# skipperro/selkies-gstreamer

Hardware: AMD Instinct MI355X
Metric: encoded fps + glass-to-glass p50 ms at 1920x1080; concurrent 60fps sessions/node (higher is better)
Workload: dtype uint8 pixels / int32 integer transforms (bit-exact vs CPU reference); 1 GPU; model=H.264 Constrained Baseline CAVLC, striped stripes 64px, CRF 25, global_batch=8, seq_len=1, parallelism=session-parallel dp1 x 8 sessions/GPU, resolution=1920x1080, backend=hip, deblock=auto, me_full=True, upload_overlap=False, frames_in_flight=1, num_refs=1, numa_node_rank0=0

## Files before the change

### csrc/kernels/h264_gpu.h

```cpp
#pragma once
#include <hip/hip_runtime.h>
#include "../codec/overlay.h"
#include "../codec/h264_encoder.h"
#include "../codec/h264_frame.h"
#include "../codec/h264_deblock.h"

namespace sk {
namespace h264 {
namespace gpu {

constexpr int kMbSlotBytes = 1024;
constexpr int kSliceHdrMax = 64;

struct Planes {
    uint8_t* y;
    uint8_t* u;
    uint8_t* v;
};

struct FrameArgs {
    int W, H, mb_w, mb_h, stride_y, stride_c, num_slices, rows_per_slice, fullframe;
    int full_range, me_range, me_iters;
    const uint8_t* bgrx;
    int bgrx_stride;
// ... 7 lines not shown
    int* plan_ctl;
    const int* key_seq_host;
    int* key_dev;
    PlanConfig plan_cfg;
    SliceTask* tasks;
    MeResult* me;
    int16_t* mvfield;
    MbInfo* mbs;
    int16_t* coefs;
    uint32_t* mb_bits;
    int* mb_nbits;
    uint32_t* rbsp;
    int rbsp_slot_words;
    int* mb_off;
    int* slice_info;
    int* tile_nz;
    int* tile_ins;
    int max_tiles;
    int out_slot_bytes;
    const uint8_t* param_sets;
    const int* param_set_len;
    int param_set_stride;
    uint8_t* host_out;
    int* host_size;
    int* frame_params_dev;
    const int* frame_params_host;
    SliceTask* tasks_host;
    unsigned long long* dbg;
    const CavlcTables* cavlc_tabs;
    int num_refs;
    int deblock;
// ... 32 lines not shown
```

### csrc/kernels/h264_kernels.hip

```cpp
#include "h264_gpu.h"
#include "../codec/color.h"
#include "../codec/h264_mb.h"

namespace sk {
namespace h264 {
namespace gpu {

__device__ __forceinline__ int lane_id() { return threadIdx.x & 63; }

__device__ __forceinline__ void wave_sync() {
    __builtin_amdgcn_fence(__ATOMIC_RELEASE, "wavefront");
    __builtin_amdgcn_wave_barrier();
    __builtin_amdgcn_fence(__ATOMIC_ACQUIRE, "wavefront");
}

__device__ __forceinline__ int wave_sum(int v) {
    v += __builtin_amdgcn_mov_dpp(v, 0xB1, 0xF, 0xF, false);
    v += __builtin_amdgcn_mov_dpp(v, 0x4E, 0xF, 0xF, false);
    v += __builtin_amdgcn_mov_dpp(v, 0x124, 0xF, 0xF, false);
    v += __builtin_amdgcn_mov_dpp(v, 0x128, 0xF, 0xF, false);
    return __builtin_amdgcn_readlane(v, 0) + __builtin_amdgcn_readlane(v, 16) +
           __builtin_amdgcn_readlane(v, 32) + __builtin_amdgcn_readlane(v, 48);
}

// ... 313 lines not shown

__device__ __forceinline__ uint32_t load_ref4(const uint8_t* row, int x, int stride) {
    if (x >= 0 && x + 3 <= stride - 1) {
        int xa = x & ~3, sh = x & 3;
        uint32_t w0 = *reinterpret_cast<const uint32_t*>(row + xa);
        if (sh == 0) return w0;
        uint32_t w1 = *reinterpret_cast<const uint32_t*>(row + xa + 4);
        return __builtin_amdgcn_alignbyte(w1, w0, sh);
    }
    uint32_t v = 0;
#pragma unroll
    for (int i = 0; i < 4; i++) v |= (uint32_t)row[sk_clip(x + i, 0, stride - 1)] << (8 * i);
    return v;
}

__device__ __forceinline__ int me_sad(const FrameArgs& a, const uint8_t* refy, uint32_t sw, int mbx,
                                      int mby, int dx, int dy, int ylo, int yhi) {
    int l = lane_id();
    int row = l >> 2, col4 = (l & 3) * 4;
    int sy = sk_clip(mby * 16 + row + dy, ylo, yhi);
    uint32_t rw = load_ref4(refy + (size_t)sy * a.stride_y, mbx * 16 + col4 + dx, a.stride_y);
    return wave_sum((int)__builtin_amdgcn_sad_u8(sw, rw, 0u));
}

constexpr int kWin = 8;
constexpr int kWinWords = 10;

__device__ __forceinline__ uint32_t win_sad_lane(const uint32_t* win, uint32_t sw, int ox, int oy) {
    const int l = lane_id();
    const int row = l >> 2, col4 = (l & 3) * 4;
    const int bc = col4 + ox + kWin;
    const uint32_t* w = win + (row + oy + kWin) * kWinWords + (bc >> 2);
    const int sh = bc & 3;
    const uint32_t rw = sh ? __builtin_amdgcn_alignbyte(w[1], w[0], sh) : w[0];
    return __builtin_amdgcn_sad_u8(sw, rw, 0u);
}

__device__ __forceinline__ int win_sad(const uint32_t* win, uint32_t sw, int ox, int oy) {
    const int l = lane_id();
    const int row = l >> 2, col4 = (l & 3) * 4;
    const int bc = col4 + ox + kWin;
    const uint32_t* w = win + (row + oy + kWin) * kWinWords + (bc >> 2);
    const int sh = bc & 3;
    const uint32_t rw = sh ? __builtin_amdgcn_alignbyte(w[1], w[0], sh) : w[0];
    return wave_sum((int)__builtin_amdgcn_sad_u8(sw, rw, 0u));
}

__device__ __forceinline__ int mb_activity(uint32_t sw) {
    const int psum = (int)(sw & 255) + (int)((sw >> 8) & 255) + (int)((sw >> 16) & 255) + (int)(sw >> 24);
    const int mean = (wave_sum(psum) + 128) >> 8;
    int dev = 0;
#pragma unroll
    for (int i = 0; i < 4; i++) dev += sk_abs((int)((sw >> (8 * i)) & 255) - mean);
    return wave_sum(dev);
}

__global__ __launch_bounds__(64) void k_motion_search(FrameArgs a) {
    __shared__ uint32_t win[32 * kWinWords];
    int nmb = a.mb_w * a.mb_h;
    int idx = xcd_remap(blockIdx.x, gridDim.x);
    if (idx >= nmb) return;
    int mbx = idx % a.mb_w, mby = idx / a.mb_w;
    int s = mby / a.rows_per_slice;
    const SliceTask t = a.tasks[s];
    if (t.action != ACT_P && t.action != ACT_I) return;
    int l = lane_id();
    int row = l >> 2, col4 = (l & 3) * 4;
    uint32_t sw = *reinterpret_cast<const uint32_t*>(a.src.y + (size_t)(mby * 16 + row) * a.stride_y +
                                                     mbx * 16 + col4);
    if (t.action == ACT_I) {
        const int dev = mb_activity(sw);
        if (l == 0) a.me[idx] = MeResult{0, 0, 0, dev, 0, 0, 0};
        return;
    }
    int ylo = t.pic_row0 * 16, yhi = (t.pic_row0 + t.pic_rows) * 16 - 1;
    const int lam = lambda_for_qp(rc_me_qp(*a.rc, t.qp));
    const int R = a.me_range;
    int cx[7], cy[7], n = 0;
    cx[0] = 0; cy[0] = 0; n = 1;
    auto add = [&](int ox, int oy) {
        int j = oy * a.mb_w + ox;
        cx[n] = sk_clip(a.mvfield[2 * j], -R, R);
        cy[n] = sk_clip(a.mvfield[2 * j + 1], -R, R);
        n++;
    };
    add(mbx, mby);
    if (mbx > 0) add(mbx - 1, mby);
    if (mbx + 1 < a.mb_w) add(mbx + 1, mby);
    if (mby - 1 >= t.pic_row0) add(mbx, mby - 1);
    if (mby + 1 < t.pic_row0 + t.pic_rows) add(mbx, mby + 1);
    if (a.me_full && a.mb_dirty[idx]) {
        cx[n] = sk_clip(a.fs_mv[2 * idx], -R, R);
        cy[n] = sk_clip(a.fs_mv[2 * idx + 1], -R, R);
        n++;
    }
    int bx = 0, by = 0;
    int bsad = me_sad(a, a.ref.y, sw, mbx, mby, 0, 0, ylo, yhi);
    int bcost = bsad + lam * (sk_se_bits(0) + sk_se_bits(0));
    for (int i = 1; i < n; i++) {
        int sd = me_sad(a, a.ref.y, sw, mbx, mby, cx[i], cy[i], ylo, yhi);
        int c = sd + lam * (sk_se_bits(4 * cx[i]) + sk_se_bits(4 * cy[i]));
        if (c < bcost) { bcost = c; bx = cx[i]; by = cy[i]; bsad = sd; }
    }
    const int cx0 = bx, cy0 = by;
    {
        const int r = l >> 1, h = l & 1;
        const int y = sk_clip(mby * 16 + cy0 - kWin + r, ylo, yhi);
        const uint8_t* rowp = a.ref.y + (size_t)y * a.stride_y;
        const int x0 = mbx * 16 + cx0 - kWin + 16 * h;
#pragma unroll
        for (int k = 0; k < 5; k++) win[r * kWinWords + 4 * h + k] = load_ref4(rowp, x0 + 4 * k, a.stride_y);
    }
    wave_sync();
    const int ddx[4] = {0, -1, 1, 0}, ddy[4] = {-1, 0, 0, 1};
    for (int it = 0; it < a.me_iters; it++) {
        int nb = -1, ncost = bcost, nsad = 0;
        bool all_in = true;
#pragma unroll
        for (int k = 0; k < 4; k++) {
            const int ox = bx + ddx[k] - cx0, oy = by + ddy[k] - cy0;
            all_in = all_in && ox >= -kWin && ox <= kWin && oy >= -kWin && oy <= kWin;
        }
        if (all_in) {
            uint32_t p[4];
#pragma unroll
            for (int k = 0; k < 4; k++) p[k] = win_sad_lane(win, sw, bx + ddx[k] - cx0, by + ddy[k] - cy0);
            const uint32_t s01 = (uint32_t)wave_sum((int)(p[0] | (p[1] << 16)));
            const uint32_t s23 = (uint32_t)wave_sum((int)(p[2] | (p[3] << 16)));
            const int sds[4] = {(int)(s01 & 0xffff), (int)(s01 >> 16), (int)(s23 & 0xffff), (int)(s23 >> 16)};
#pragma unroll
            for (int k = 0; k < 4; k++) {
                int x = bx + ddx[k], y = by + ddy[k];
                if (x < -R || x > R || y < -R || y > R) continue;
                int c = sds[k] + lam * (sk_se_bits(4 * x) + sk_se_bits(4 * y));
                if (c < ncost) { ncost = c; nb = k; nsad = sds[k]; }
            }
            if (nb < 0) break;
            bx += ddx[nb]; by += ddy[nb]; bcost = ncost; bsad = nsad;
            continue;
        }
#pragma unroll
        for (int k = 0; k < 4; k++) {
            int x = bx + ddx[k], y = by + ddy[k];
            if (x < -R || x > R || y < -R || y > R) continue;
            const int ox = x - cx0, oy = y - cy0;
            int sd = (ox >= -kWin && ox <= kWin && oy >= -kWin && oy <= kWin)
                         ? win_sad(win, sw, ox, oy)
                         : me_sad(a, a.ref.y, sw, mbx, mby, x, y, ylo, yhi);
            int c = sd + lam * (sk_se_bits(4 * x) + sk_se_bits(4 * y));
            if (c < ncost) { ncost = c; nb = k; nsad = sd; }
        }
        if (nb < 0) break;
        bx += ddx[nb]; by += ddy[nb]; bcost = ncost; bsad = nsad;
    }
    const int dev = mb_activity(sw);
    int refi = 0;
    if (t.num_refs > 1 && a.mb_dirty[idx]) {
        const int s1 = me_sad(a, a.ref1.y, sw, mbx, mby, 0, 0, ylo, yhi);
        if (s1 + 3 * lam < bcost) {
            bx = by = 0;
            bsad = s1;
            refi = 1;
        }
    }
    if (l == 0) {
        MeResult r;
        r.mvx = (int16_t)bx;
        r.mvy = (int16_t)by;
        r.sad = bsad;
        r.intra_est = dev;
        r.ref = (int16_t)refi;
        r.fx = r.fy = 0;
        a.me[idx] = r;
    }
}

typedef int v4i __attribute__((ext_vector_type(4)));

__global__ __launch_bounds__(256) void k_me_mfma(FrameArgs a) {
    constexpr int WW = kFsWin / 4;
    constexpr int WP = WW + 1;
    constexpr int BP = 5;
    constexpr int SP = 2 * kFsR + 4;
    __shared__ uint32_t win_s[4][kFsWin * WP];
    __shared__ uint32_t blk_s[4][16 * BP];
    __shared__ __align__(16) int sq_s[4][kFsWin * SP];
    const int w = threadIdx.x >> 6, l = lane_id();
    const int nmb = a.mb_w * a.mb_h;
    const int idx = xcd_remap(blockIdx.x, gridDim.x) * 4 + w;
    if (idx >= nmb) return;
    const int mbx = idx % a.mb_w, mby = idx / a.mb_w;
    const SliceTask t = a.tasks[mby / a.rows_per_slice];
    if (t.action != ACT_P || !a.mb_dirty[idx]) return;
    const int ylo = t.pic_row0 * 16, yhi = (t.pic_row0 + t.pic_rows) * 16 - 1;
    {
        const int R = a.me_range;
        const int px = sk_clip(a.mvfield[2 * idx], -R, R), py = sk_clip(a.mvfield[2 * idx + 1], -R, R);
        const uint32_t sw = *reinterpret_cast<const uint32_t*>(a.src.y + (size_t)(mby * 16 + (l >> 2)) * a.stride_y +
                                                               mbx * 16 + (l & 3) * 4);
        if (me_sad(a, a.ref.y, sw, mbx, mby, px, py, ylo, yhi) == 0) {
            if (l == 0) {
                a.fs_mv[2 * idx] = (int16_t)px;
                a.fs_mv[2 * idx + 1] = (int16_t)py;
            }
            return;
        }
    }
    uint32_t* win = win_s[w];
    uint32_t* blk = blk_s[w];
    int* sq = sq_s[w];
    for (int i = l; i < kFsWin * WW; i += 64) {
        const int wy = i / WW, q = i - wy * WW;
        const int y = sk_clip(mby * 16 - kFsR + wy, ylo, yhi);
        win[wy * WP + q] = load_ref4(a.ref.y + (size_t)y * a.stride_y, mbx * 16 - kFsR + 4 * q, a.stride_y);
    }
    blk[(l >> 2) * BP + (l & 3)] = *reinterpret_cast<const uint32_t*>(a.src.y + (size_t)(mby * 16 + (l >> 2)) * a.stride_y +
                                                                     mbx * 16 + (l & 3) * 4);
    wave_sync();
    if (l < kFsWin) {
        uint32_t rw[WW];
#pragma unroll
        for (int q = 0; q < WW; q++) rw[q] = win[l * WP + q];
        int sqv[kFsWin];
#pragma unroll
        for (int c = 0; c < kFsWin; c++) {
            const int v = (int)((rw[c >> 2] >> (8 * (c & 3))) & 255) - 128;
            sqv[c] = v * v;
        }
        int acc = 0;
#pragma unroll
        for (int c = 0; c < 16; c++) acc += sqv[c];
        int out[2 * kFsR];
        out[0] = acc;
#pragma unroll
        for (int x = 1; x < 2 * kFsR; x++) {
            acc += sqv[x + 15] - sqv[x - 1];
            out[x] = acc;
        }
#pragma unroll
        for (int x = 0; x < 2 * kFsR; x += 4)
            *reinterpret_cast<int4*>(&sq[l * SP + x]) = make_int4(out[x], out[x + 1], out[x + 2], out[x + 3]);
    }
    wave_sync();
    if (l < 2 * kFsR) {
        int col[kFsWin];
#pragma unroll
        for (int r = 0; r < kFsWin; r++) col[r] = sq[r * SP + l];
        int acc = 0;
#pragma unroll
        for (int r = 0; r < 16; r++) acc += col[r];
#pragma unroll
        for (int dy = 0; dy < 2 * kFsR; dy++) {
            sq[dy * SP + l] = acc;
            acc += col[dy + 16] - col[dy];
        }
    }
    const int i16 = l & 15, g = l >> 4;
    v4i acc[2][2];
#pragma unroll
    for (int mt = 0; mt < 2; mt++)
#pragma unroll
        for (int nt = 0; nt < 2; nt++) acc[mt][nt] = v4i{0, 0, 0, 0};
#pragma unroll
    for (int ks = 0; ks < kFsWin / 4; ks++) {
        const int rr = 4 * ks + g;
        v4i bf[2];
#pragma unroll
        for (int nt = 0; nt < 2; nt++) {
            const int src = rr - (16 * nt + i16);
            const bool in = src >= 0 && src < 16;
#pragma unroll
            for (int q = 0; q < 4; q++) bf[nt][q] = in ? (int)(blk[(in ? src : 0) * BP + q] ^ 0x80808080u) : 0;
        }
#pragma unroll
        for (int mt = 0; mt < 2; mt++) {
            const int b0 = 16 * mt + i16;
            const uint32_t* wr = win + rr * WP + (b0 >> 2);
            const int sh = b0 & 3;
            uint32_t w5[5];
#pragma unroll
            for (int q = 0; q < 5; q++) w5[q] = wr[q];
            v4i af;
#pragma unroll
            for (int q = 0; q < 4; q++) af[q] = (int)(__builtin_amdgcn_alignbyte(w5[q + 1], w5[q], sh) ^ 0x80808080u);
#pragma unroll
            for (int nt = 0; nt < 2; nt++)
                if (ks >= 4 * nt && ks <= 4 * nt + 7)
                    acc[mt][nt] = __builtin_amdgcn_mfma_i32_16x16x64_i8(af, bf[nt], acc[mt][nt], 0, 0, 0);
        }
    }
    wave_sync();
    uint64_t best = ~0ull;
#pragma unroll
    for (int mt = 0; mt < 2; mt++)
#pragma unroll
        for (int nt = 0; nt < 2; nt++) {
            const int dyw = 16 * nt + i16;
            const int4 sv = *reinterpret_cast<const int4*>(&sq[dyw * SP + 16 * mt + 4 * g]);
            const int svr[4] = {sv.x, sv.y, sv.z, sv.w};
#pragma unroll
            for (int reg = 0; reg < 4; reg++) {
                const int dxw = 16 * mt + 4 * g + reg;
                const uint64_t k = fs_key(svr[reg] - 2 * acc[mt][nt][reg], dyw, dxw);
                best = k < best ? k : best;
            }
        }
#pragma unroll
    for (int o = 1; o < 64; o <<= 1) {
        const uint64_t other = __shfl_xor(best, o);
        best = other < best ? other : best;
    }
    if (l == 0) {
        a.fs_mv[2 * idx] = (int16_t)fs_key_dx(best);
        a.fs_mv[2 * idx + 1] = (int16_t)fs_key_dy(best);
    }
}

__global__ __launch_bounds__(256) void k_plan(FrameArgs a) {
    const int ns = a.num_slices, tid = threadIdx.x;
    StripeState* st = a.plan_state;
    StripeState& pic = st[ns];
    if (a.plan_ctl[1] == 1) {
        if (a.fullframe) {
            bool idr = true;
            for (int s = tid; s < ns; s += 256) idr &= a.tasks[s].final_action == ACT_I && a.tasks[s].idr_on_intra;
            idr = __syncthreads_and(idr);
            if (tid == 0) commit_picture(pic, idr, a.plan_cfg.num_refs);
        } else {
            for (int s = tid; s < ns; s += 256) commit_stripe(st[s], a.tasks[s].final_action, a.plan_cfg.num_refs);
        }
// ... 88 lines not shown
                rc.last_bits[k] = old.last_bits[k];
                rc.last_cplx[k] = old.last_cplx[k];
            }
        if (old.mode == mode) rc.cplx_ema = old.cplx_ema;
        rc.seq = seq;
    }
    rc.base_qp = plan_qp;
    rc_apply(rc, a.tasks, a.rc_slice, a.rc_slice + 1, a.num_slices, a.mb_w, plan_qp, 2);
}
__global__ __launch_bounds__(64) void k_rc_qp(FrameArgs a) {
    if (threadIdx.x == 0) rc_qp_serial(a);
    __syncthreads();
    for (int s = threadIdx.x; s < a.num_slices; s += 64) a.tasks_host[s].qp = a.tasks[s].qp;
}

__global__ __launch_bounds__(64) void k_rc_account(FrameArgs a, const int* sizes, int n, int stride, int per_slice) {
    long long b = 0;
    for (int i = threadIdx.x; i < n; i += 64)
        if (!per_slice || i % per_slice < slice_nals(a, a.tasks[i / per_slice])) b += sizes[(size_t)i * stride];
    for (int o = 32; o > 0; o >>= 1) b += __shfl_down(b, o);
    if (threadIdx.x == 0) rc_account(*a.rc, 8 * b);
}

__global__ __launch_bounds__(256) void k_rc_guard(FrameArgs a) {
    __shared__ long long part[4];
    const int s = blockIdx.x, tid = threadIdx.x;
    long long b = 0;
    for (int i = tid; i < a.num_slices; i += 256) {
        const int nn = slice_nals(a, a.tasks[i]);
        for (int j = 0; j < nn; j++) b += a.slice_info[4 * (i * a.nal_per_slice + j)];
    }
    for (int o = 32; o > 0; o >>= 1) b += __shfl_down(b, o);
    if ((tid & 63) == 0) part[tid >> 6] = b;
    __syncthreads();
    const long long bits = 8 * (part[0] + part[1] + part[2] + part[3]);
    const int step = rc_redo_step(*a.rc, bits);
// ... 1654 lines not shown
            uint32_t hi = 0u;
            if (k >= 1) {
                hi = src[k - 1];
                if (k - 1 == nw - 1) hi &= lastmask;
            }
            v = (lo >> sh) | (k >= 1 ? hi << (32 - sh) : 0u);
        }
        if (j == w0 || j == w1) {
            if (v) atomicOr(&dst[j], v);
        } else {
            dst[j] = v;
        }
    }
}

__device__ __forceinline__ uint8_t rbsp_byte(uint32_t word, int q) { return (uint8_t)(word >> (24 - 8 * q)); }

__global__ __launch_bounds__(256) void k_ep_nz(FrameArgs a) {
    __shared__ int red[4];
    const int s = blockIdx.y, t = blockIdx.x, tid = threadIdx.x;
    const int nn = slice_nals(a, a.tasks[s]);
    for (int j = 0; j < nn; j++) {
    const int nal = s * a.nal_per_slice + j;
    const int n = a.slice_info[4 * nal];
    const int t0 = t * kTile;
    if (t0 >= n) continue;
    const uint32_t* rbsp = nal_rbsp(a, s, j);
    const int i0 = t0 + tid * 16;
    int lastnz = -1;
#pragma unroll
    for (int q = 0; q < 4; q++) {
        const int iq = i0 + 4 * q;
        const uint32_t wd = iq < n ? rbsp[iq >> 2] : 0u;
#pragma unroll
        for (int b = 0; b < 4; b++)
            if (iq + b < n && rbsp_byte(wd, b)) lastnz = iq + b;
    }
    for (int o = 32; o > 0; o >>= 1) lastnz = max(lastnz, __shfl_down(lastnz, o));
    if (lane_id() == 0) red[tid >> 6] = lastnz;
    __syncthreads();
    if (tid == 0) a.tile_nz[nal * a.max_tiles + t] = max(max(red[0], red[1]), max(red[2], red[3]));
    __syncthreads();
    }
}

__device__ __forceinline__ int ep_thread(const uint32_t* rbsp, int n, int t0, int carry, int* scan_lds,
                                         uint8_t* by, uint32_t* insmask) {
    const int tid = threadIdx.x, wv = tid >> 6, ln = tid & 63;
    const int i0 = t0 + tid * 16;
    int lastnz = -1;
#pragma unroll
    for (int q = 0; q < 4; q++) {
        const int iq = i0 + 4 * q;
        const uint32_t wd = iq < n ? rbsp[iq >> 2] : 0u;
#pragma unroll
        for (int j = 0; j < 4; j++) {
            by[4 * q + j] = rbsp_byte(wd, j);
            if (iq + j < n && by[4 * q + j]) lastnz = iq + j;
        }
    }
    const int incl = wave_incl_scan_max(lastnz);
    int ex = __shfl_up(incl, 1);
    if (ln == 0) ex = -1;
    if (ln == 63) scan_lds[wv] = incl;
    __syncthreads();
    int prev = carry;
    for (int k = 0; k < wv; k++) prev = max(prev, scan_lds[k]);
    prev = max(prev, ex);
    int ins = 0;
    uint32_t mask = 0;
#pragma unroll
    for (int q = 0; q < 16; q++) {
        const int i = i0 + q;
        if (i < n) {
            const int z = i - 1 - prev;
            if (by[q] <= 3 && z >= 2 && !(z & 1)) {
                ins++;
                mask |= 1u << q;
            }
            if (by[q]) prev = i;
        }
    }
    *insmask = mask;
    return ins;
}

__device__ __forceinline__ int tile_carry(const FrameArgs& a, int nal, int t) {
    int c = -1;
    for (int k = 0; k < t; k++) c = max(c, a.tile_nz[nal * a.max_tiles + k]);
    return c;
}

__global__ __launch_bounds__(256) void k_ep_count(FrameArgs a) {
    __shared__ int scan_lds[4];
    __shared__ int red[4];
    const int s = blockIdx.y, t = blockIdx.x;
    const int nn = slice_nals(a, a.tasks[s]);
    for (int j = 0; j < nn; j++) {
        const int nal = s * a.nal_per_slice + j;
        const int n = a.slice_info[4 * nal];
        const int t0 = t * kTile;
        if (t0 >= n) continue;
        const uint32_t* rbsp = nal_rbsp(a, s, j);
        uint8_t by[16];
        uint32_t mask;
        int ins = ep_thread(rbsp, n, t0, tile_carry(a, nal, t), scan_lds, by, &mask);
        for (int o = 32; o > 0; o >>= 1) ins += __shfl_down(ins, o);
        if (lane_id() == 0) red[threadIdx.x >> 6] = ins;
        __syncthreads();
        if (threadIdx.x == 0) a.tile_ins[nal * a.max_tiles + t] = red[0] + red[1] + red[2] + red[3];
        __syncthreads();
    }
}

__global__ __launch_bounds__(256) void k_ep_write(FrameArgs a) {
    __shared__ int scan_lds[4];
    __shared__ int wave_tot[5];
    __shared__ int sh_before, sh_base;
    __shared__ uint8_t sOut[kTile + kTile / 2 + 16];
    const int s = blockIdx.y, t = blockIdx.x, tid = threadIdx.x;
    const SliceTask& task = a.tasks[s];
// ... 10 lines not shown
        int base = 0;
        for (int jj = 0; jj < j; jj++) {
            const int q = s * a.nal_per_slice + jj, nq = a.slice_info[4 * q];
            int ins_q = 0;
            for (int k = tid; k * kTile < nq; k += 64) ins_q += a.tile_ins[q * a.max_tiles + k];
            base += a.slice_info[4 * q + 1] + nq + wave_sum(ins_q);
        }
        if (tid == 0) {
            sh_before = b;
            sh_base = base;
        }
    }
    uint32_t* rbsp = nal_rbsp(a, s, j);
    uint8_t by[16];
    uint32_t mask;
    const int ins = ep_thread(rbsp, n, t0, tile_carry(a, nal, t), scan_lds, by, &mask);
    int tile_ins;
    const int ex = block_excl_scan<4>(ins, wave_tot, &tile_ins);
    const int i0 = t0 + tid * 16;
    int o = tid * 16 + ex;
#pragma unroll
    for (int q = 0; q < 16; q++) {
        if (i0 + q < n) {
            if (mask & (1u << q)) sOut[o++] = 3;
            sOut[o++] = by[q];
        }
    }
#pragma unroll
    for (int q = 0; q < 4; q++)
        if (i0 + 4 * q < n) rbsp[(i0 >> 2) + q] = 0u;
    __syncthreads();
// ... 319 lines not shown
            }
        }
        lds_barrier();
    }
}

void launch_convert_damage(const FrameArgs& a, hipStream_t s) {
    dim3 grid((a.mb_w + 15) / 16, a.mb_h);
    if (a.yuv_fmt) hipLaunchKernelGGL(k_yuv_damage, grid, dim3(256), 0, s, a);
    else hipLaunchKernelGGL(k_convert_damage, grid, dim3(256), 0, s, a);
}

void launch_frontend(const FrameArgs& a, hipStream_t s) {
    int nmb = a.mb_w * a.mb_h;
    hipLaunchKernelGGL(k_plan, dim3(1), dim3(256), 0, s, a);
    if (a.me_full) hipLaunchKernelGGL(k_me_mfma, dim3((nmb + 3) / 4), dim3(256), 0, s, a);
    hipLaunchKernelGGL(k_motion_search, dim3(nmb), dim3(64), 0, s, a);
    hipLaunchKernelGGL(k_decide, dim3(a.num_slices), dim3(256), 0, s, a);
    hipLaunchKernelGGL(k_rc_qp, dim3(1), dim3(64), 0, s, a);
    if (a.subpel) hipLaunchKernelGGL(k_subpel, dim3((nmb + 3) / 4), dim3(256), 0, s, a);
}

void launch_rc_guard_sizes(const FrameArgs& a, const int* sizes, int n, int* redo, bool chained, hipStream_t s) {
    hipLaunchKernelGGL(k_rc_guard_sizes, dim3(1), dim3(256), 0, s, a, sizes, n, redo, chained ? 1 : 0);
}

void launch_rc_account(const FrameArgs& a, const int* sizes, int n, int stride, int per_slice, hipStream_t s) {
    hipLaunchKernelGGL(k_rc_account, dim3(1), dim3(64), 0, s, a, sizes, n, stride, per_slice);
}

static void launch_code(const FrameArgs& a, hipStream_t s) {
    int nmb = a.mb_w * a.mb_h;
// ... 10 lines not shown
}

void launch_encode(const FrameArgs& a, hipStream_t s, bool guard) {
    int nmb = a.mb_w * a.mb_h;
    launch_frontend(a, s);
    if (a.aq_strength > 0) hipLaunchKernelGGL(k_aq, dim3((nmb + 3) / 4), dim3(256), 0, s, a);
    launch_code(a, s);
    if (guard && a.rc_redo) {
        hipLaunchKernelGGL(k_rc_guard, dim3(a.num_slices), dim3(256), 0, s, a);
        FrameArgs b = a;
        b.gate = a.rc_redo;
        launch_code(b, s);
    }
    hipLaunchKernelGGL(k_mb_concat, dim3((nmb + 3) / 4), dim3(256), 0, s, a);
    const dim3 tiles(a.max_tiles, a.num_slices);
    hipLaunchKernelGGL(k_ep_nz, tiles, dim3(256), 0, s, a);
    hipLaunchKernelGGL(k_ep_count, tiles, dim3(256), 0, s, a);
    hipLaunchKernelGGL(k_ep_write, tiles, dim3(256), 0, s, a);
    launch_rc_account(a, a.slice_info, a.num_slices * a.nal_per_slice, 4, a.nal_per_slice, s);
}

void launch_commit(const FrameArgs& a, hipStream_t s) {
    hipLaunchKernelGGL(k_commit, dim3((a.mb_w + 15) / 16, a.mb_h), dim3(256), 0, s, a);
    if (a.deblock) {
        const int nmb = a.mb_w * a.mb_h;
        hipLaunchKernelGGL(k_deblock_prep, dim3((nmb + 3) / 4), dim3(256), 0, s, a);
        hipLaunchKernelGGL(k_deblock_edges, dim3((nmb + 255) / 256), dim3(256), 0, s, a);
        if (a.rows_per_slice <= 4)
            hipLaunchKernelGGL(k_deblock<4>, dim3(a.num_slices), dim3(64 * a.rows_per_slice), 0, s, a);
        else
            hipLaunchKernelGGL(k_deblock<kMaxRows>, dim3(a.num_slices), dim3(64 * a.rows_per_slice), 0, s, a);
    }
}

// ... 4 lines not shown
```

### csrc/runtime/h264_hip.cpp

```cpp
#include "encoder_iface.h"
#include "trace.h"
#include "../kernels/h264_gpu.h"
#include "../kernels/hevc_gpu.h"
#include "../kernels/av1_gpu.h"
#include "../codec/av1_encoder.h"
#include "../kernels/runtime_kernels.h"
#include "../codec/hevc_encoder.h"
#include <hip/hip_runtime.h>
#include <atomic>
#include <chrono>
#include <map>
#include <mutex>
#include <stdexcept>
#include <string.h>
#include <string>
#include <thread>
#include <vector>
#include <atomic>

namespace sk {
namespace {

#define HIPCHECK(x)                                                                     \
    do {                                                                                \
// ... 530 lines not shown
        a.dbe = dmalloc<uint4>((size_t)3 * nmb);
        a.mbs = dmalloc<MbInfo>(nmb);
        a.coefs = dmalloc<int16_t>((size_t)nmb * kCoefPerMb);
        a.mb_bits = dmalloc<uint32_t>((size_t)nmb * (gpu::kMbSlotBytes / 4));
        a.mb_nbits = dmalloc<int>(nmb);
        int max_slice_mbs = g_.rows_per_slice * g_.mb_w;
        const bool can_split = cfg_.codec == 0 && g_.mb_w > kIntraSubMbs;
        a.nal_per_slice = can_split ? max_nals_per_slice(g_.rows_per_slice, g_.mb_w) : 1;
        a.sub_rbsp_words = (kIntraSubMbs * gpu::kMbSlotBytes + 1024) / 4;
        a.rbsp_slot_words = std::max((max_slice_mbs * gpu::kMbSlotBytes + 1024) / 4,
                                     can_split ? a.nal_per_slice * a.sub_rbsp_words : 0);
        a.rbsp = dmalloc<uint32_t>((size_t)ns * a.rbsp_slot_words);
        a.mb_off = dmalloc<int>(nmb);
        a.slice_info = dmalloc<int>(4 * (size_t)ns * a.nal_per_slice);
        a.max_tiles = (a.rbsp_slot_words * 4 + 4095) / 4096;
        a.tile_nz = dmalloc<int>((size_t)ns * a.nal_per_slice * a.max_tiles);
        a.tile_ins = dmalloc<int>((size_t)ns * a.nal_per_slice * a.max_tiles);
        size_t slot = ((size_t)a.rbsp_slot_words * 4 * 3 / 2 + 1024 + 63) & ~(size_t)63;
        a.out_slot_bytes = (int)slot;
        void* dptr = nullptr;
        for (int p = 0; p < 2; p++) {
            host_out_[p] = hmalloc<uint8_t>(slot * ns);
            h_out_size_[p] = hmalloc<int>(ns);
            HIPCHECK(hipHostGetDevicePointer(&dptr, host_out_[p], 0));
            host_out_dev_[p] = (uint8_t*)dptr;
            HIPCHECK(hipHostGetDevicePointer(&dptr, h_out_size_[p], 0));
            host_size_dev_[p] = (int*)dptr;
        }
        std::vector<std::vector<uint8_t>> ps;
        if (cfg_.fullframe) {
            ps.resize(1);
// ... 475 lines not shown
```

Before: 5109 frames/s (1920x1080 H.264, all sessions, all GPUs).

## Fuse full-search and motion refinement into one ME kernel; drop ep_nz pass

Merges the MFMA full-search kernel and the diamond motion-search kernel into a single k_me kernel. The refinement reuses the large full-search window in LDS and batches candidate SADs into paired wave reductions. The emulation-prevention pass loses its separate nonzero-scan kernel: each tile now finds its carry by a ballot scan backwards over the RBSP. The rate-control accounting launch is folded into k_ep_count. These changes cut kernel launches, global round-trips and redundant reference loads, at the cost of a more complex kernel with possibly higher register and LDS use and a serial backwards carry scan per tile.

```diff
diff --git a/csrc/codec/h264_ep.h b/csrc/codec/h264_ep.h
--- /dev/null
+++ b/csrc/codec/h264_ep.h
@@ -0,0 +1,25 @@
+#pragma once
+#include "sk_common.h"
+
+namespace sk {
+namespace h264 {
+
+SK_HD uint8_t ep_rbsp_byte(uint32_t word, int q) { return (uint8_t)(word >> (24 - 8 * q)); }
+
+SK_HD int ep_last_nz_in_word(uint32_t word) { return 3 - (__builtin_ctz(word) >> 3); }
+
+template <class Ballot>
+SK_HD int ep_tile_carry(const uint32_t* rbsp, int t0, int lane, int nlanes, Ballot ballot) {
+    for (int top = (t0 >> 2) - 1; top >= 0; top -= nlanes) {
+        const int wi = top - lane;
+        const uint64_t m = ballot(wi >= 0 && rbsp[wi] != 0u);
+        if (m) {
+            const int f = top - __builtin_ctzll(m);
+            return 4 * f + ep_last_nz_in_word(rbsp[f]);
+        }
+    }
+    return -1;
+}
+
+}
+}
diff --git a/csrc/kernels/h264_gpu.h b/csrc/kernels/h264_gpu.h
--- a/csrc/kernels/h264_gpu.h
+++ b/csrc/kernels/h264_gpu.h
@@ -45,7 +45,7 @@
     int rbsp_slot_words;
     int* mb_off;
     int* slice_info;
-    int* tile_nz;
+    int* tile_carry;
     int* tile_ins;
     int max_tiles;
     int out_slot_bytes;
diff --git a/csrc/kernels/h264_kernels.hip b/csrc/kernels/h264_kernels.hip
--- a/csrc/kernels/h264_kernels.hip
+++ b/csrc/kernels/h264_kernels.hip
@@ -1,6 +1,7 @@
 #include "h264_gpu.h"
 #include "../codec/color.h"
 #include "../codec/h264_mb.h"
+#include "../codec/h264_ep.h"
 
 namespace sk {
 namespace h264 {
@@ -351,36 +352,42 @@
     return v;
 }
 
-__device__ __forceinline__ int me_sad(const FrameArgs& a, const uint8_t* refy, uint32_t sw, int mbx,
-                                      int mby, int dx, int dy, int ylo, int yhi) {
+__device__ __forceinline__ uint32_t me_sad_lane(const FrameArgs& a, const uint8_t* refy, uint32_t sw, int mbx,
+                                                int mby, int dx, int dy, int ylo, int yhi) {
     int l = lane_id();
     int row = l >> 2, col4 = (l & 3) * 4;
     int sy = sk_clip(mby * 16 + row + dy, ylo, yhi);
     uint32_t rw = load_ref4(refy + (size_t)sy * a.stride_y, mbx * 16 + col4 + dx, a.stride_y);
-    return wave_sum((int)__builtin_amdgcn_sad_u8(sw, rw, 0u));
+    return __builtin_amdgcn_sad_u8(sw, rw, 0u);
+}
+
+__device__ __forceinline__ int me_sad(const FrameArgs& a, const uint8_t* refy, uint32_t sw, int mbx,
+                                      int mby, int dx, int dy, int ylo, int yhi) {
+    return wave_sum((int)me_sad_lane(a, refy, sw, mbx, mby, dx, dy, ylo, yhi));
 }
 
 constexpr int kWin = 8;
 constexpr int kWinWords = 10;
-
-__device__ __forceinline__ uint32_t win_sad_lane(const uint32_t* win, uint32_t sw, int ox, int oy) {
+constexpr int kFsWinWords = kFsWin / 4 + 1;
+
+struct MeWin {
+    const uint32_t* w;
+    int stride;
+    int rad;
+    int cx, cy;
+    __device__ __forceinline__ bool has(int dx, int dy) const {
+        return dx - cx >= -rad && dx - cx <= rad && dy - cy >= -rad && dy - cy <= rad;
+    }
+};
+
+__device__ __forceinline__ uint32_t win_sad_lane(const MeWin& wn, uint32_t sw, int dx, int dy) {
     const int l = lane_id();
     const int row = l >> 2, col4 = (l & 3) * 4;
-    const int bc = col4 + ox + kWin;
-    const uint32_t* w = win + (row + oy + kWin) * kWinWords + (bc >> 2);
+    const int bc = col4 + dx - wn.cx + wn.rad;
+    const uint32_t* w = wn.w + (row + dy - wn.cy + wn.rad) * wn.stride + (bc >> 2);
     const int sh = bc & 3;
     const uint32_t rw = sh ? __builtin_amdgcn_alignbyte(w[1], w[0], sh) : w[0];
     return __builtin_amdgcn_sad_u8(sw, rw, 0u);
-}
-
-__device__ __forceinline__ int win_sad(const uint32_t* win, uint32_t sw, int ox, int oy) {
-    const int l = lane_id();
-    const int row = l >> 2, col4 = (l & 3) * 4;
-    const int bc = col4 + ox + kWin;
-    const uint32_t* w = win + (row + oy + kWin) * kWinWords + (bc >> 2);
-    const int sh = bc & 3;
-    const uint32_t rw = sh ? __builtin_amdgcn_alignbyte(w[1], w[0], sh) : w[0];
-    return wave_sum((int)__builtin_amdgcn_sad_u8(sw, rw, 0u));
 }
 
 __device__ __forceinline__ int mb_activity(uint32_t sw) {
@@ -392,100 +399,91 @@
     return wave_sum(dev);
 }
 
-__global__ __launch_bounds__(64) void k_motion_search(FrameArgs a) {
-    __shared__ uint32_t win[32 * kWinWords];
-    int nmb = a.mb_w * a.mb_h;
-    int idx = xcd_remap(blockIdx.x, gridDim.x);
-    if (idx >= nmb) return;
-    int mbx = idx % a.mb_w, mby = idx / a.mb_w;
-    int s = mby / a.rows_per_slice;
-    const SliceTask t = a.tasks[s];
-    if (t.action != ACT_P && t.action != ACT_I) return;
-    int l = lane_id();
-    int row = l >> 2, col4 = (l & 3) * 4;
-    uint32_t sw = *reinterpret_cast<const uint32_t*>(a.src.y + (size_t)(mby * 16 + row) * a.stride_y +
-                                                     mbx * 16 + col4);
+__device__ __forceinline__ void me_search_mb(const FrameArgs& a, const SliceTask& t, int idx, int mbx, int mby,
+                                             uint32_t sw, bool have_fs, int fsx, int fsy, uint32_t* win, bool big) {
+    const int l = lane_id();
     if (t.action == ACT_I) {
         const int dev = mb_activity(sw);
         if (l == 0) a.me[idx] = MeResult{0, 0, 0, dev, 0, 0, 0};
         return;
     }
-    int ylo = t.pic_row0 * 16, yhi = (t.pic_row0 + t.pic_rows) * 16 - 1;
+    const int ylo = t.pic_row0 * 16, yhi = (t.pic_row0 + t.pic_rows) * 16 - 1;
     const int lam = lambda_for_qp(rc_me_qp(*a.rc, t.qp));
     const int R = a.me_range;
-    int cx[7], cy[7], n = 0;
-    cx[0] = 0; cy[0] = 0; n = 1;
-    auto add = [&](int ox, int oy) {
-        int j = oy * a.mb_w + ox;
-        cx[n] = sk_clip(a.mvfield[2 * j], -R, R);
-        cy[n] = sk_clip(a.mvfield[2 * j + 1], -R, R);
-        n++;
+    MeWin wn{win, big ? kFsWinWords : kWinWords, big ? kFsR : -1, 0, 0};
+    auto sad_lane = [&](int dx, int dy) {
+        return wn.has(dx, dy) ? win_sad_lane(wn, sw, dx, dy) : me_sad_lane(a, a.ref.y, sw, mbx, mby, dx, dy, ylo, yhi);
     };
-    add(mbx, mby);
-    if (mbx > 0) add(mbx - 1, mby);
-    if (mbx + 1 < a.mb_w) add(mbx + 1, mby);
-    if (mby - 1 >= t.pic_row0) add(mbx, mby - 1);
-    if (mby + 1 < t.pic_row0 + t.pic_rows) add(mbx, mby + 1);
-    if (a.me_full && a.mb_dirty[idx]) {
-        cx[n] = sk_clip(a.fs_mv[2 * idx], -R, R);
-        cy[n] = sk_clip(a.fs_mv[2 * idx + 1], -R, R);
-        n++;
+    int cx[7], cy[7];
+    bool ok[7];
+    auto slot = [&](int k, bool valid, int ox, int oy) {
+        const int j = valid ? oy * a.mb_w + ox : idx;
+        ok[k] = valid;
+        cx[k] = sk_clip(a.mvfield[2 * j], -R, R);
+        cy[k] = sk_clip(a.mvfield[2 * j + 1], -R, R);
+    };
+    cx[0] = 0; cy[0] = 0; ok[0] = true;
+    slot(1, true, mbx, mby);
+    slot(2, mbx > 0, mbx - 1, mby);
+    slot(3, mbx + 1 < a.mb_w, mbx + 1, mby);
+    slot(4, mby - 1 >= t.pic_row0, mbx, mby - 1);
+    slot(5, mby + 1 < t.pic_row0 + t.pic_rows, mbx, mby + 1);
+    ok[6] = have_fs;
+    cx[6] = sk_clip(fsx, -R, R);
+    cy[6] = sk_clip(fsy, -R, R);
+    int sd[8];
+    {
+        uint32_t p[8];
+#pragma unroll
+        for (int k = 0; k < 7; k++) p[k] = ok[k] ? sad_lane(cx[k], cy[k]) : 0u;
+        p[7] = 0u;
+#pragma unroll
+        for (int k = 0; k < 8; k += 2) {
+            const uint32_t s2 = (uint32_t)wave_sum((int)(p[k] | (p[k + 1] << 16)));
+            sd[k] = (int)(s2 & 0xffff);
+            sd[k + 1] = (int)(s2 >> 16);
+        }
     }
     int bx = 0, by = 0;
-    int bsad = me_sad(a, a.ref.y, sw, mbx, mby, 0, 0, ylo, yhi);
+    int bsad = sd[0];
     int bcost = bsad + lam * (sk_se_bits(0) + sk_se_bits(0));
-    for (int i = 1; i < n; i++) {
-        int sd = me_sad(a, a.ref.y, sw, mbx, mby, cx[i], cy[i], ylo, yhi);
-        int c = sd + lam * (sk_se_bits(4 * cx[i]) + sk_se_bits(4 * cy[i]));
-        if (c < bcost) { bcost = c; bx = cx[i]; by = cy[i]; bsad = sd; }
-    }
-    const int cx0 = bx, cy0 = by;
-    {
+#pragma unroll
+    for (int k = 1; k < 7; k++) {
+        if (!ok[k]) continue;
+        int c = sd[k] + lam * (sk_se_bits(4 * cx[k]) + sk_se_bits(4 * cy[k]));
+        if (c < bcost) { bcost = c; bx = cx[k]; by = cy[k]; bsad = sd[k]; }
+    }
+    if (!(big && wn.has(bx, by))) {
+        wave_sync();
         const int r = l >> 1, h = l & 1;
-        const int y = sk_clip(mby * 16 + cy0 - kWin + r, ylo, yhi);
+        const int y = sk_clip(mby * 16 + by - kWin + r, ylo, yhi);
         const uint8_t* rowp = a.ref.y + (size_t)y * a.stride_y;
-        const int x0 = mbx * 16 + cx0 - kWin + 16 * h;
+        const int x0 = mbx * 16 + bx - kWin + 16 * h;
 #pragma unroll
         for (int k = 0; k < 5; k++) win[r * kWinWords + 4 * h + k] = load_ref4(rowp, x0 + 4 * k, a.stride_y);
-    }
-    wave_sync();
+        wn = MeWin{win, kWinWords, kWin, bx, by};
+        wave_sync();
+    }
     const int ddx[4] = {0, -1, 1, 0}, ddy[4] = {-1, 0, 0, 1};
     for (int it = 0; it < a.me_iters; it++) {
+        uint32_t p[4];
+        bool in_r[4];
+#pragma unroll
+        for (int k = 0; k < 4; k++) {
+            const int x = bx + ddx[k], y = by + ddy[k];
+            in_r[k] = !(x < -R || x > R || y < -R || y > R);
+            p[k] = in_r[k] ? sad_lane(x, y) : 0u;
+        }
+        const uint32_t s01 = (uint32_t)wave_sum((int)(p[0] | (p[1] << 16)));
+        const uint32_t s23 = (uint32_t)wave_sum((int)(p[2] | (p[3] << 16)));
+        const int sds[4] = {(int)(s01 & 0xffff), (int)(s01 >> 16), (int)(s23 & 0xffff), (int)(s23 >> 16)};
         int nb = -1, ncost = bcost, nsad = 0;
-        bool all_in = true;
 #pragma unroll
         for (int k = 0; k < 4; k++) {
-            const int ox = bx + ddx[k] - cx0, oy = by + ddy[k] - cy0;
-            all_in = all_in && ox >= -kWin && ox <= kWin && oy >= -kWin && oy <= kWin;
-        }
-        if (all_in) {
-            uint32_t p[4];
-#pragma unroll
-            for (int k = 0; k < 4; k++) p[k] = win_sad_lane(win, sw, bx + ddx[k] - cx0, by + ddy[k] - cy0);
-            const uint32_t s01 = (uint32_t)wave_sum((int)(p[0] | (p[1] << 16)));
-            const uint32_t s23 = (uint32_t)wave_sum((int)(p[2] | (p[3] << 16)));
-            const int sds[4] = {(int)(s01 & 0xffff), (int)(s01 >> 16), (int)(s23 & 0xffff), (int)(s23 >> 16)};
-#pragma unroll
-            for (int k = 0; k < 4; k++) {
-                int x = bx + ddx[k], y = by + ddy[k];
-                if (x < -R || x > R || y < -R || y > R) continue;
-                int c = sds[k] + lam * (sk_se_bits(4 * x) + sk_se_bits(4 * y));
-                if (c < ncost) { ncost = c; nb = k; nsad = sds[k]; }
-            }
-            if (nb < 0) break;
-            bx += ddx[nb]; by += ddy[nb]; bcost = ncost; bsad = nsad;
-            continue;
-        }
-#pragma unroll
-        for (int k = 0; k < 4; k++) {
+            if (!in_r[k]) continue;
             int x = bx + ddx[k], y = by + ddy[k];
-            if (x < -R || x > R || y < -R || y > R) continue;
-            const int ox = x - cx0, oy = y - cy0;
-            int sd = (ox >= -kWin && ox <= kWin && oy >= -kWin && oy <= kWin)
-                         ? win_sad(win, sw, ox, oy)
-                         : me_sad(a, a.ref.y, sw, mbx, mby, x, y, ylo, yhi);
-            int c = sd + lam * (sk_se_bits(4 * x) + sk_se_bits(4 * y));
-            if (c < ncost) { ncost = c; nb = k; nsad = sd; }
+            int c = sds[k] + lam * (sk_se_bits(4 * x) + sk_se_bits(4 * y));
+            if (c < ncost) { ncost = c; nb = k; nsad = sds[k]; }
         }
         if (nb < 0) break;
         bx += ddx[nb]; by += ddy[nb]; bcost = ncost; bsad = nsad;
@@ -512,145 +510,173 @@
     }
 }
 
+__global__ __launch_bounds__(64) void k_motion_search(FrameArgs a) {
+    __shared__ uint32_t win[32 * kWinWords];
+    int nmb = a.mb_w * a.mb_h;
+    int idx = xcd_remap(blockIdx.x, gridDim.x);
+    if (idx >= nmb) return;
+    int mbx = idx % a.mb_w, mby = idx / a.mb_w;
+    const SliceTask t = a.tasks[mby / a.rows_per_slice];
+    if (t.action != ACT_P && t.action != ACT_I) return;
+    int l = lane_id();
+    uint32_t sw = *reinterpret_cast<const uint32_t*>(a.src.y + (size_t)(mby * 16 + (l >> 2)) * a.stride_y +
+                                                     mbx * 16 + (l & 3) * 4);
+    const bool have_fs = a.me_full && t.action == ACT_P && a.mb_dirty[idx];
+    const int fsx = have_fs ? a.fs_mv[2 * idx] : 0, fsy = have_fs ? a.fs_mv[2 * idx + 1] : 0;
+    me_search_mb(a, t, idx, mbx, mby, sw, have_fs, fsx, fsy, win, false);
+}
+
 typedef int v4i __attribute__((ext_vector_type(4)));
 
-__global__ __launch_bounds__(256) void k_me_mfma(FrameArgs a) {
+constexpr int kFsBlkWords = 5;
+constexpr int kFsSqInts = 2 * kFsR + 4;
+
+__device__ __forceinline__ uint64_t fs_search(const FrameArgs& a, uint32_t* win, uint32_t* blk, int* sq, int mbx, int mby,
+                                              uint32_t sw, int ylo, int yhi) {
     constexpr int WW = kFsWin / 4;
-    constexpr int WP = WW + 1;
-    constexpr int BP = 5;
-    constexpr int SP = 2 * kFsR + 4;
-    __shared__ uint32_t win_s[4][kFsWin * WP];
-    __shared__ uint32_t blk_s[4][16 * BP];
-    __shared__ __align__(16) int sq_s[4][kFsWin * SP];
+    constexpr int WP = kFsWinWords;
+    constexpr int BP = kFsBlkWords;
+    constexpr int SP = kFsSqInts;
+    const int l = lane_id();
+    for (int i = l; i < kFsWin * WW; i += 64) {
+        const int wy = i / WW, q = i - wy * WW;
+        const int y = sk_clip(mby * 16 - kFsR + wy, ylo, yhi);
+        win[wy * WP + q] = load_ref4(a.ref.y + (size_t)y * a.stride_y, mbx * 16 - kFsR + 4 * q, a.stride_y);
+    }
+    blk[(l >> 2) * BP + (l & 3)] = sw;
+    wave_sync();
+    if (l < kFsWin) {
+        uint32_t rw[WW];
+#pragma unroll
+        for (int q = 0; q < WW; q++) rw[q] = win[l * WP + q];
+        int sqv[kFsWin];
+#pragma unroll
+        for (int c = 0; c < kFsWin; c++) {
+            const int v = (int)((rw[c >> 2] >> (8 * (c & 3))) & 255) - 128;
+            sqv[c] = v * v;
+        }
+        int acc = 0;
+#pragma unroll
+        for (int c = 0; c < 16; c++) acc += sqv[c];
+        int out[2 * kFsR];
+        out[0] = acc;
+#pragma unroll
+        for (int x = 1; x < 2 * kFsR; x++) {
+            acc += sqv[x + 15] - sqv[x - 1];
+            out[x] = acc;
+        }
+#pragma unroll
+        for (int x = 0; x < 2 * kFsR; x += 4)
+            *reinterpret_cast<int4*>(&sq[l * SP + x]) = make_int4(out[x], out[x + 1], out[x + 2], out[x + 3]);
+    }
+    wave_sync();
+    if (l < 2 * kFsR) {
+        int col[kFsWin];
+#pragma unroll
+        for (int r = 0; r < kFsWin; r++) col[r] = sq[r * SP + l];
+        int acc = 0;
+#pragma unroll
+        for (int r = 0; r < 16; r++) acc += col[r];
+#pragma unroll
+        for (int dy = 0; dy < 2 * kFsR; dy++) {
+            sq[dy * SP + l] = acc;
+            acc += col[dy + 16] - col[dy];
+        }
+    }
+    const int i16 = l & 15, g = l >> 4;
+    v4i acc[2][2];
+#pragma unroll
+    for (int mt = 0; mt < 2; mt++)
+#pragma unroll
+        for (int nt = 0; nt < 2; nt++) acc[mt][nt] = v4i{0, 0, 0, 0};
+#pragma unroll
+    for (int ks = 0; ks < kFsWin / 4; ks++) {
+        const int rr = 4 * ks + g;
+        v4i bf[2];
+#pragma unroll
+        for (int nt = 0; nt < 2; nt++) {
+            const int src = rr - (16 * nt + i16);
+            const bool in = src >= 0 && src < 16;
+#pragma unroll
+            for (int q = 0; q < 4; q++) bf[nt][q] = in ? (int)(blk[(in ? src : 0) * BP + q] ^ 0x80808080u) : 0;
+        }
+#pragma unroll
+        for (int mt = 0; mt < 2; mt++) {
+            const int b0 = 16 * mt + i16;
+            const uint32_t* wr = win + rr * WP + (b0 >> 2);
+            const int sh = b0 & 3;
+            uint32_t w5[5];
+#pragma unroll
+            for (int q = 0; q < 5; q++) w5[q] = wr[q];
+            v4i af;
+#pragma unroll
+            for (int q = 0; q < 4; q++) af[q] = (int)(__builtin_amdgcn_alignbyte(w5[q + 1], w5[q], sh) ^ 0x80808080u);
+#pragma unroll
+            for (int nt = 0; nt < 2; nt++)
+                if (ks >= 4 * nt && ks <= 4 * nt + 7)
+                    acc[mt][nt] = __builtin_amdgcn_mfma_i32_16x16x64_i8(af, bf[nt], acc[mt][nt], 0, 0, 0);
+        }
+    }
+    wave_sync();
+    uint64_t best = ~0ull;
+#pragma unroll
+    for (int mt = 0; mt < 2; mt++)
+#pragma unroll
+        for (int nt = 0; nt < 2; nt++) {
+            const int dyw = 16 * nt + i16;
+            const int4 sv = *reinterpret_cast<const int4*>(&sq[dyw * SP + 16 * mt + 4 * g]);
+            const int svr[4] = {sv.x, sv.y, sv.z, sv.w};
+#pragma unroll
+            for (int reg = 0; reg < 4; reg++) {
+                const int dxw = 16 * mt + 4 * g + reg;
+                const uint64_t k = fs_key(svr[reg] - 2 * acc[mt][nt][reg], dyw, dxw);
+                best = k < best ? k : best;
+            }
+        }
+#pragma unroll
+    for (int o = 1; o < 64; o <<= 1) {
+        const uint64_t other = __shfl_xor(best, o);
+        best = other < best ? other : best;
+    }
+    return best;
+}
+
+__global__ __launch_bounds__(256) void k_me(FrameArgs a) {
+    __shared__ uint32_t win_s[4][kFsWin * kFsWinWords];
+    __shared__ uint32_t blk_s[4][16 * kFsBlkWords];
+    __shared__ __align__(16) int sq_s[4][kFsWin * kFsSqInts];
+    static_assert(kFsWin * kFsWinWords >= 32 * kWinWords, "the small window lives in the wave's win_s region");
     const int w = threadIdx.x >> 6, l = lane_id();
     const int nmb = a.mb_w * a.mb_h;
     const int idx = xcd_remap(blockIdx.x, gridDim.x) * 4 + w;
     if (idx >= nmb) return;
     const int mbx = idx % a.mb_w, mby = idx / a.mb_w;
     const SliceTask t = a.tasks[mby / a.rows_per_slice];
-    if (t.action != ACT_P || !a.mb_dirty[idx]) return;
-    const int ylo = t.pic_row0 * 16, yhi = (t.pic_row0 + t.pic_rows) * 16 - 1;
-    {
+    if (t.action != ACT_P && t.action != ACT_I) return;
+    const uint32_t sw = *reinterpret_cast<const uint32_t*>(a.src.y + (size_t)(mby * 16 + (l >> 2)) * a.stride_y +
+                                                           mbx * 16 + (l & 3) * 4);
+    bool have_fs = false, big = false;
+    int fsx = 0, fsy = 0;
+    if (t.action == ACT_P && a.mb_dirty[idx]) {
+        have_fs = true;
+        const int ylo = t.pic_row0 * 16, yhi = (t.pic_row0 + t.pic_rows) * 16 - 1;
         const int R = a.me_range;
         const int px = sk_clip(a.mvfield[2 * idx], -R, R), py = sk_clip(a.mvfield[2 * idx + 1], -R, R);
-        const uint32_t sw = *reinterpret_cast<const uint32_t*>(a.src.y + (size_t)(mby * 16 + (l >> 2)) * a.stride_y +
-                                                               mbx * 16 + (l & 3) * 4);
         if (me_sad(a, a.ref.y, sw, mbx, mby, px, py, ylo, yhi) == 0) {
-            if (l == 0) {
-                a.fs_mv[2 * idx] = (int16_t)px;
-                a.fs_mv[2 * idx + 1] = (int16_t)py;
-            }
-            return;
-        }
-    }
-    uint32_t* win = win_s[w];
-    uint32_t* blk = blk_s[w];
-    int* sq = sq_s[w];
-    for (int i = l; i < kFsWin * WW; i += 64) {
-        const int wy = i / WW, q = i - wy * WW;
-        const int y = sk_clip(mby * 16 - kFsR + wy, ylo, yhi);
-        win[wy * WP + q] = load_ref4(a.ref.y + (size_t)y * a.stride_y, mbx * 16 - kFsR + 4 * q, a.stride_y);
-    }
-    blk[(l >> 2) * BP + (l & 3)] = *reinterpret_cast<const uint32_t*>(a.src.y + (size_t)(mby * 16 + (l >> 2)) * a.stride_y +
-                                                                     mbx * 16 + (l & 3) * 4);
-    wave_sync();
-    if (l < kFsWin) {
-        uint32_t rw[WW];
-#pragma unroll
-        for (int q = 0; q < WW; q++) rw[q] = win[l * WP + q];
-        int sqv[kFsWin];
-#pragma unroll
-        for (int c = 0; c < kFsWin; c++) {
-            const int v = (int)((rw[c >> 2] >> (8 * (c & 3))) & 255) - 128;
-            sqv[c] = v * v;
-        }
-        int acc = 0;
-#pragma unroll
-        for (int c = 0; c < 16; c++) acc += sqv[c];
-        int out[2 * kFsR];
-        out[0] = acc;
-#pragma unroll
-        for (int x = 1; x < 2 * kFsR; x++) {
-            acc += sqv[x + 15] - sqv[x - 1];
-            out[x] = acc;
-        }
-#pragma unroll
-        for (int x = 0; x < 2 * kFsR; x += 4)
-            *reinterpret_cast<int4*>(&sq[l * SP + x]) = make_int4(out[x], out[x + 1], out[x + 2], out[x + 3]);
-    }
-    wave_sync();
-    if (l < 2 * kFsR) {
-        int col[kFsWin];
-#pragma unroll
-        for (int r = 0; r < kFsWin; r++) col[r] = sq[r * SP + l];
-        int acc = 0;
-#pragma unroll
-        for (int r = 0; r < 16; r++) acc += col[r];
-#pragma unroll
-        for (int dy = 0; dy < 2 * kFsR; dy++) {
-            sq[dy * SP + l] = acc;
-            acc += col[dy + 16] - col[dy];
-        }
-    }
-    const int i16 = l & 15, g = l >> 4;
-    v4i acc[2][2];
-#pragma unroll
-    for (int mt = 0; mt < 2; mt++)
-#pragma unroll
-        for (int nt = 0; nt < 2; nt++) acc[mt][nt] = v4i{0, 0, 0, 0};
-#pragma unroll
-    for (int ks = 0; ks < kFsWin / 4; ks++) {
-        const int rr = 4 * ks + g;
-        v4i bf[2];
-#pragma unroll
-        for (int nt = 0; nt < 2; nt++) {
-            const int src = rr - (16 * nt + i16);
-            const bool in = src >= 0 && src < 16;
-#pragma unroll
-            for (int q = 0; q < 4; q++) bf[nt][q] = in ? (int)(blk[(in ? src : 0) * BP + q] ^ 0x80808080u) : 0;
-        }
-#pragma unroll
-        for (int mt = 0; mt < 2; mt++) {
-            const int b0 = 16 * mt + i16;
-            const uint32_t* wr = win + rr * WP + (b0 >> 2);
-            const int sh = b0 & 3;
-            uint32_t w5[5];
-#pragma unroll
-            for (int q = 0; q < 5; q++) w5[q] = wr[q];
-            v4i af;
-#pragma unroll
-            for (int q = 0; q < 4; q++) af[q] = (int)(__builtin_amdgcn_alignbyte(w5[q + 1], w5[q], sh) ^ 0x80808080u);
-#pragma unroll
-            for (int nt = 0; nt < 2; nt++)
-                if (ks >= 4 * nt && ks <= 4 * nt + 7)
-                    acc[mt][nt] = __builtin_amdgcn_mfma_i32_16x16x64_i8(af, bf[nt], acc[mt][nt], 0, 0, 0);
-        }
-    }
-    wave_sync();
-    uint64_t best = ~0ull;
-#pragma unroll
-    for (int mt = 0; mt < 2; mt++)
-#pragma unroll
-        for (int nt = 0; nt < 2; nt++) {
-            const int dyw = 16 * nt + i16;
-            const int4 sv = *reinterpret_cast<const int4*>(&sq[dyw * SP + 16 * mt + 4 * g]);
-            const int svr[4] = {sv.x, sv.y, sv.z, sv.w};
-#pragma unroll
-            for (int reg = 0; reg < 4; reg++) {
-                const int dxw = 16 * mt + 4 * g + reg;
-                const uint64_t k = fs_key(svr[reg] - 2 * acc[mt][nt][reg], dyw, dxw);
-                best = k < best ? k : best;
-            }
-        }
-#pragma unroll
-    for (int o = 1; o < 64; o <<= 1) {
-        const uint64_t other = __shfl_xor(best, o);
-        best = other < best ? other : best;
-    }
-    if (l == 0) {
-        a.fs_mv[2 * idx] = (int16_t)fs_key_dx(best);
-        a.fs_mv[2 * idx + 1] = (int16_t)fs_key_dy(best);
-    }
+            fsx = px;
+            fsy = py;
+        } else {
+            const uint64_t best = fs_search(a, win_s[w], blk_s[w], sq_s[w], mbx, mby, sw, ylo, yhi);
+            fsx = __builtin_amdgcn_readfirstlane(fs_key_dx(best));
+            fsy = __builtin_amdgcn_readfirstlane(fs_key_dy(best));
+            big = true;
+        }
+        if (l == 0) {
+            a.fs_mv[2 * idx] = (int16_t)fsx;
+            a.fs_mv[2 * idx + 1] = (int16_t)fsy;
+        }
+    }
+    me_search_mb(a, t, idx, mbx, mby, sw, have_fs, fsx, fsy, win_s[w], big);
 }
 
 __global__ __launch_bounds__(256) void k_plan(FrameArgs a) {
@@ -769,12 +795,16 @@
     for (int s = threadIdx.x; s < a.num_slices; s += 64) a.tasks_host[s].qp = a.tasks[s].qp;
 }
 
-__global__ __launch_bounds__(64) void k_rc_account(FrameArgs a, const int* sizes, int n, int stride, int per_slice) {
+__device__ __forceinline__ void rc_account_wave(const FrameArgs& a, const int* sizes, int n, int stride, int per_slice) {
     long long b = 0;
-    for (int i = threadIdx.x; i < n; i += 64)
+    for (int i = lane_id(); i < n; i += 64)
         if (!per_slice || i % per_slice < slice_nals(a, a.tasks[i / per_slice])) b += sizes[(size_t)i * stride];
     for (int o = 32; o > 0; o >>= 1) b += __shfl_down(b, o);
-    if (threadIdx.x == 0) rc_account(*a.rc, 8 * b);
+    if (lane_id() == 0) rc_account(*a.rc, 8 * b);
+}
+
+__global__ __launch_bounds__(64) void k_rc_account(FrameArgs a, const int* sizes, int n, int stride, int per_slice) {
+    rc_account_wave(a, sizes, n, stride, per_slice);
 }
 
 __global__ __launch_bounds__(256) void k_rc_guard(FrameArgs a) {
@@ -2459,37 +2489,10 @@
     }
 }
 
-__device__ __forceinline__ uint8_t rbsp_byte(uint32_t word, int q) { return (uint8_t)(word >> (24 - 8 * q)); }
-
-__global__ __launch_bounds__(256) void k_ep_nz(FrameArgs a) {
-    __shared__ int red[4];
-    const int s = blockIdx.y, t = blockIdx.x, tid = threadIdx.x;
-    const int nn = slice_nals(a, a.tasks[s]);
-    for (int j = 0; j < nn; j++) {
-    const int nal = s * a.nal_per_slice + j;
-    const int n = a.slice_info[4 * nal];
-    const int t0 = t * kTile;
-    if (t0 >= n) continue;
-    const uint32_t* rbsp = nal_rbsp(a, s, j);
-    const int i0 = t0 + tid * 16;
-    int lastnz = -1;
-#pragma unroll
-    for (int q = 0; q < 4; q++) {
-        const int iq = i0 + 4 * q;
-        const uint32_t wd = iq < n ? rbsp[iq >> 2] : 0u;
-#pragma unroll
-        for (int b = 0; b < 4; b++)
-            if (iq + b < n && rbsp_byte(wd, b)) lastnz = iq + b;
-    }
-    for (int o = 32; o > 0; o >>= 1) lastnz = max(lastnz, __shfl_down(lastnz, o));
-    if (lane_id() == 0) red[tid >> 6] = lastnz;
-    __syncthreads();
-    if (tid == 0) a.tile_nz[nal * a.max_tiles + t] = max(max(red[0], red[1]), max(red[2], red[3]));
-    __syncthreads();
-    }
-}
-
-__device__ __forceinline__ int ep_thread(const uint32_t* rbsp, int n, int t0, int carry, int* scan_lds,
+__device__ __forceinline__ uint8_t rbsp_byte(uint32_t word, int q) { return ep_rbsp_byte(word, q); }
+
+template <class Carry>
+__device__ __forceinline__ int ep_thread(const uint32_t* rbsp, int n, int t0, Carry carry, int* scan_lds,
                                          uint8_t* by, uint32_t* insmask) {
     const int tid = threadIdx.x, wv = tid >> 6, ln = tid & 63;
     const int i0 = t0 + tid * 16;
@@ -2509,7 +2512,7 @@
     if (ln == 0) ex = -1;
     if (ln == 63) scan_lds[wv] = incl;
     __syncthreads();
-    int prev = carry;
+    int prev = carry();
     for (int k = 0; k < wv; k++) prev = max(prev, scan_lds[k]);
     prev = max(prev, ex);
     int ins = 0;
@@ -2530,16 +2533,13 @@
     return ins;
 }
 
-__device__ __forceinline__ int tile_carry(const FrameArgs& a, int nal, int t) {
-    int c = -1;
-    for (int k = 0; k < t; k++) c = max(c, a.tile_nz[nal * a.max_tiles + k]);
-    return c;
-}
-
 __global__ __launch_bounds__(256) void k_ep_count(FrameArgs a) {
     __shared__ int scan_lds[4];
     __shared__ int red[4];
+    __shared__ int sh_carry;
     const int s = blockIdx.y, t = blockIdx.x;
+    if (s == 0 && t == 0 && threadIdx.x < 64)
+        rc_account_wave(a, a.slice_info, a.num_slices * a.nal_per_slice, 4, a.nal_per_slice);
     const int nn = slice_nals(a, a.tasks[s]);
     for (int j = 0; j < nn; j++) {
         const int nal = s * a.nal_per_slice + j;
@@ -2547,9 +2547,16 @@
         const int t0 = t * kTile;
         if (t0 >= n) continue;
         const uint32_t* rbsp = nal_rbsp(a, s, j);
+        if (threadIdx.x < 64) {
+            const int c = ep_tile_carry(rbsp, t0, lane_id(), 64, [](bool p) { return (uint64_t)__ballot(p); });
+            if (threadIdx.x == 0) {
+                sh_carry = c;
+                a.tile_carry[nal * a.max_tiles + t] = c;
+            }
+        }
         uint8_t by[16];
         uint32_t mask;
-        int ins = ep_thread(rbsp, n, t0, tile_carry(a, nal, t), scan_lds, by, &mask);
+        int ins = ep_thread(rbsp, n, t0, [&] { return sh_carry; }, scan_lds, by, &mask);
         for (int o = 32; o > 0; o >>= 1) ins += __shfl_down(ins, o);
         if (lane_id() == 0) red[threadIdx.x >> 6] = ins;
         __syncthreads();
@@ -2590,7 +2597,8 @@
     uint32_t* rbsp = nal_rbsp(a, s, j);
     uint8_t by[16];
     uint32_t mask;
-    const int ins = ep_thread(rbsp, n, t0, tile_carry(a, nal, t), scan_lds, by, &mask);
+    const int carry = a.tile_carry[nal * a.max_tiles + t];
+    const int ins = ep_thread(rbsp, n, t0, [&] { return carry; }, scan_lds, by, &mask);
     int tile_ins;
     const int ex = block_excl_scan<4>(ins, wave_tot, &tile_ins);
     const int i0 = t0 + tid * 16;
@@ -2940,8 +2948,8 @@
 void launch_frontend(const FrameArgs& a, hipStream_t s) {
     int nmb = a.mb_w * a.mb_h;
     hipLaunchKernelGGL(k_plan, dim3(1), dim3(256), 0, s, a);
-    if (a.me_full) hipLaunchKernelGGL(k_me_mfma, dim3((nmb + 3) / 4), dim3(256), 0, s, a);
-    hipLaunchKernelGGL(k_motion_search, dim3(nmb), dim3(64), 0, s, a);
+    if (a.me_full) hipLaunchKernelGGL(k_me, dim3((nmb + 3) / 4), dim3(256), 0, s, a);
+    else hipLaunchKernelGGL(k_motion_search, dim3(nmb), dim3(64), 0, s, a);
     hipLaunchKernelGGL(k_decide, dim3(a.num_slices), dim3(256), 0, s, a);
     hipLaunchKernelGGL(k_rc_qp, dim3(1), dim3(64), 0, s, a);
     if (a.subpel) hipLaunchKernelGGL(k_subpel, dim3((nmb + 3) / 4), dim3(256), 0, s, a);
@@ -2982,10 +2990,8 @@
     }
     hipLaunchKernelGGL(k_mb_concat, dim3((nmb + 3) / 4), dim3(256), 0, s, a);
     const dim3 tiles(a.max_tiles, a.num_slices);
-    hipLaunchKernelGGL(k_ep_nz, tiles, dim3(256), 0, s, a);
     hipLaunchKernelGGL(k_ep_count, tiles, dim3(256), 0, s, a);
     hipLaunchKernelGGL(k_ep_write, tiles, dim3(256), 0, s, a);
-    launch_rc_account(a, a.slice_info, a.num_slices * a.nal_per_slice, 4, a.nal_per_slice, s);
 }
 
 void launch_commit(const FrameArgs& a, hipStream_t s) {
diff --git a/csrc/runtime/h264_hip.cpp b/csrc/runtime/h264_hip.cpp
--- a/csrc/runtime/h264_hip.cpp
+++ b/csrc/runtime/h264_hip.cpp
@@ -568,7 +568,7 @@
         a.mb_off = dmalloc<int>(nmb);
         a.slice_info = dmalloc<int>(4 * (size_t)ns * a.nal_per_slice);
         a.max_tiles = (a.rbsp_slot_words * 4 + 4095) / 4096;
-        a.tile_nz = dmalloc<int>((size_t)ns * a.nal_per_slice * a.max_tiles);
+        a.tile_carry = dmalloc<int>((size_t)ns * a.nal_per_slice * a.max_tiles);
         a.tile_ins = dmalloc<int>((size_t)ns * a.nal_per_slice * a.max_tiles);
         size_t slot = ((size_t)a.rbsp_slot_words * 4 * 3 / 2 + 1024 + 63) & ~(size_t)63;
         a.out_slot_bytes = (int)slot;
```

Result: faster. 5596 frames/s (1920x1080 H.264, all sessions, all GPUs) (median of 6 runs) (+9.5%).
